# VISION-SJTU/UniDefense

Measured on AMD Instinct MI355X. Metric: images/sec fwd+bwd (256x256, EffNet-b4), higher is better.
Workload: dtype f32

## Files before the change

unidefense_amd/csrc/gemm_p3.hip:

```cpp
#include "gemm_internal.h"
#include "ud_common.h"

#include <algorithm>
#include <type_traits>

namespace {

constexpr int NT = 512;
constexpr int BK = 32;
constexpr int BM = 128, BN = 128;
constexpr int PLANE_IMG = 128 * 64;

template <int PREC> struct Cfg {
    static constexpr int NPL = PREC;
    static constexpr int OP_IMG = NPL * PLANE_IMG;
    static constexpr int STAGE = 2 * OP_IMG;
    static constexpr int NSTAGE = PREC == 3 ? 3 : 4;
    static constexpr int PT = 4 * NPL;
    static constexpr int NTERM = PREC == 3 ? 6 : PREC == 2 ? 3 : 1;
};

typedef __bf16 bf16x8 __attribute__((ext_vector_type(8)));
typedef _Float16 f16x8 __attribute__((ext_vector_type(8)));
typedef short s16x4 __attribute__((ext_vector_type(4)));
typedef short s16x8 __attribute__((ext_vector_type(8)));
typedef __attribute__((address_space(3))) char lds_char;

__device__ __forceinline__ void dma_piece(unsigned voff, unsigned lds_dst, const char* gbase) {
    unsigned keep;
    asm volatile(
        "s_nop 1\n\t"
        "s_mov_b32 %0, m0\n\t"
        "s_mov_b32 m0, %2\n\t"
// ... 10 lines not shown
}
template <int PT>
__device__ __forceinline__ void wait_tiles_and_barrier(int tiles) {
    if (tiles <= 0) wait_dma_and_barrier<0>();
    else if (tiles == 1) wait_dma_and_barrier<PT>();
    else if (tiles == 2) wait_dma_and_barrier<2 * PT>();
    else if (tiles == 3 || PT > 4) wait_dma_and_barrier<3 * PT>();
    else if (tiles == 4) wait_dma_and_barrier<4 * PT>();
    else if (tiles == 5) wait_dma_and_barrier<5 * PT>();
    else wait_dma_and_barrier<6 * PT>();
}
__device__ __forceinline__ void wait_lds_and_barrier() {
    asm volatile("s_waitcnt lgkmcnt(0)\n\ts_barrier" ::: "memory");
}

template <int NPL> struct Frags {
    s16x8 v[2][NPL];
};

template <int MODE>
struct Reader {
    unsigned b0, b1;

    __device__ __forceinline__ void init(int lane, int wrow) {
        if constexpr (MODE == 0) {
            const int r = lane & 31, h = lane >> 5, x = (r >> 2) & 3;
            b0 = (unsigned)((wrow + r) * 64 + ((h ^ x) << 4));
            b1 = (unsigned)((wrow + r) * 64 + (((2 + h) ^ x) << 4));
        } else {
            const int g = lane >> 4, u = lane & 15, q = u >> 2, pp = u & 3;
            b0 = (unsigned)((wrow >> 5) * 2048 + (8 * (g >> 1) + q) * 64 + (g & 1) * 32 + pp * 8);
            b1 = 0;
        }
    }

    template <int S, int I, int PL, int NPL>
    __device__ __forceinline__ void read_one(const lds_char* img, Frags<NPL>& f) const {
        if constexpr (MODE == 0) {
            const lds_char* p = img + (S == 0 ? b0 : b1) + I * 2048 + PL * PLANE_IMG;
            f.v[I][PL] = *reinterpret_cast<const __attribute__((address_space(3))) s16x8*>(p);
        } else {
            const lds_char* p = img + b0 + S * 1024 + I * 2048 + PL * PLANE_IMG;
            const s16x4 lo = __builtin_amdgcn_ds_read_tr16_b64_v4i16((__attribute__((address_space(3))) s16x4*)(p));
            const s16x4 hi = __builtin_amdgcn_ds_read_tr16_b64_v4i16((__attribute__((address_space(3))) s16x4*)(p + 256));
            f.v[I][PL] = __builtin_shufflevector(lo, hi, 0, 1, 2, 3, 4, 5, 6, 7);
        }
    }

    template <int S, int NPL>
    __device__ __forceinline__ void read(const lds_char* img, Frags<NPL>& f) const {
        read_one<S, 0, 0>(img, f); read_one<S, 1, 0>(img, f);
        if constexpr (NPL >= 2) { read_one<S, 0, 1>(img, f); read_one<S, 1, 1>(img, f); }
        if constexpr (NPL == 3) { read_one<S, 0, 2>(img, f); read_one<S, 1, 2>(img, f); }
    }
};

template <int MODE>
__device__ __forceinline__ unsigned dma_lane_offset(int lane) {
    if constexpr (MODE == 0) return (unsigned)((lane >> 2) * 64 + (((lane & 3) ^ ((lane >> 4) & 3)) << 4));
    else return (unsigned)(lane * 16);
}

template <int PREC, int TERM> struct Term {
    static constexpr int pa = PREC == 3 ? (TERM == 0 ? 2 : (TERM == 1 || TERM >= 4) ? 0 : 1) : PREC == 2 ? (TERM == 0 ? 1 : 0) : 0;
    static constexpr int pb = PREC == 3 ? (TERM == 0 ? 0 : TERM == 1 ? 2 : (TERM == 2 || TERM == 4) ? 1 : 0) : PREC == 2 ? (TERM == 1 ? 1 : 0) : 0;
};

template <int PREC, int Mi>
__device__ __forceinline__ void mma_one(f32x16 (&acc)[2][2], f32x16 (&lo)[2][2], const Frags<PREC>& a, const Frags<PREC>& b) {
    constexpr int term = Mi / 4, i = (Mi % 4) / 2, j = Mi % 2;
    using Tm = Term<PREC, term>;
    if constexpr (PREC == 3) {
        acc[i][j] = __builtin_amdgcn_mfma_f32_32x32x16_bf16(__builtin_bit_cast(bf16x8, a.v[i][Tm::pa]),
                                                            __builtin_bit_cast(bf16x8, b.v[j][Tm::pb]), acc[i][j], 0, 0, 0);
    } else if constexpr (PREC == 1) {
        acc[i][j] = __builtin_amdgcn_mfma_f32_32x32x16_f16(__builtin_bit_cast(f16x8, a.v[i][0]),
                                                           __builtin_bit_cast(f16x8, b.v[j][0]), acc[i][j], 0, 0, 0);
    } else if constexpr (term < 2) {
        lo[i][j] = __builtin_amdgcn_mfma_f32_32x32x16_f16(__builtin_bit_cast(f16x8, a.v[i][Tm::pa]),
                                                          __builtin_bit_cast(f16x8, b.v[j][Tm::pb]), lo[i][j], 0, 0, 0);
    } else {
        acc[i][j] = __builtin_amdgcn_mfma_f32_32x32x16_f16(__builtin_bit_cast(f16x8, a.v[i][Tm::pa]),
                                                           __builtin_bit_cast(f16x8, b.v[j][Tm::pb]), acc[i][j], 0, 0, 0);
    }
}

template <int PREC, int AMODE, int BMODE, bool SK>
__device__ __forceinline__ void p3_body(const ud_gemm_p3_desc& d, int tiles_m, int tiles_n, char* L, int bx, int by, int gx) {
    using CF = Cfg<PREC>;
    constexpr int NPL = CF::NPL, OP_IMG = CF::OP_IMG, STAGE = CF::STAGE, NSTAGE = CF::NSTAGE, PT = CF::PT;

    const int tid = threadIdx.x, lane = tid & 63;
    const int wave = __builtin_amdgcn_readfirstlane(tid >> 6);
    const int wm = (wave >> 1) & 1, wn = wave & 1;
    const int l31 = lane & 31, half = lane >> 5;
    const int kt_total = d.K / BK;
    const int dM = d.M, dN = d.N;
    const long ldc = d.ldc;
    const bool c_half = d.c_half != 0;
    double* const stat_sum = d.stat_sum;
    double* const stat_sumsq = d.stat_sumsq;
    const float* const a_inv = d.a_inv_scale;
    const float* const b_inv = d.b_inv_scale;
    const long ast = d.a_scale_stride, bst = d.b_scale_stride;
    const lds_char* Lp = (const lds_char*)L;
    const unsigned lds0 = (unsigned)(uintptr_t)Lp;
    const int lw = wave & 3;
    const unsigned dst_w = lds0 + (unsigned)lw * 2048u;
    const long a_plane = d.a_plane * 2, b_plane = d.b_plane * 2;
    const unsigned a_voff = dma_lane_offset<AMODE>(lane), b_voff = dma_lane_offset<BMODE>(lane);
    Reader<AMODE> ra;
    Reader<BMODE> rb;
    ra.init(lane, wm * 64);
    rb.init(lane, wn * 64);
    using std::integral_constant;
    using H0 = integral_constant<int, 0>;
    using H1 = integral_constant<int, 1>;
    using T = std::true_type;
    using F = std::false_type;

    auto segment = [&](int tile_m, int tile_n, int kt0, int nkt, int ep, float* Cp, bool first) {
        const int m0 = tile_m * BM, n0 = tile_n * BN;
        f32x16 acc[2][2], lo[PREC == 2 ? 2 : 1][2];
#pragma unroll
        for (int i = 0; i < 2; ++i)
#pragma unroll
            for (int j = 0; j < 2; ++j)
#pragma unroll
                for (int r = 0; r < 16; ++r) {
                    acc[i][j][r] = 0.f;
                    if constexpr (PREC == 2) lo[i][j][r] = 0.f;
                }

        if (nkt > 0) {
            if (wave >= 4) {
                const char* a_g0;
                const char* b_g0;
                long a_step, b_step;
                if constexpr (AMODE == 0) {
                    a_g0 = reinterpret_cast<const char*>(d.A) + (long)kt0 * d.a_panel * 2 + (long)(m0 + 32 * lw) * 64;
                    a_step = d.a_panel * 2;
                } else {
                    a_g0 = reinterpret_cast<const char*>(d.A) + (long)min(m0 / 32 + lw, d.a_npanel - 1) * d.a_panel * 2 +
                           (long)kt0 * BK * 64;
                    a_step = BK * 64;
                }
                if constexpr (BMODE == 0) {
                    b_g0 = reinterpret_cast<const char*>(d.B) + (long)kt0 * d.b_panel * 2 + (long)(n0 + 32 * lw) * 64;
                    b_step = d.b_panel * 2;
                } else {
                    b_g0 = reinterpret_cast<const char*>(d.B) + (long)min(n0 / 32 + lw, d.b_npanel - 1) * d.b_panel * 2 +
                           (long)kt0 * BK * 64;
                    b_step = BK * 64;
                }
                auto issue = [&](int t) {
                    const unsigned dst = dst_w + (unsigned)(t % NSTAGE) * STAGE;
                    const char* ga = a_g0 + (long)t * a_step;
                    const char* gb = b_g0 + (long)t * b_step;
#pragma unroll
                    for (int pl = 0; pl < NPL; ++pl)
#pragma unroll
                        for (int jj = 0; jj < 2; ++jj)
                            dma_piece(a_voff, dst + pl * PLANE_IMG + jj * 1024, ga + pl * a_plane + jj * 1024);
#pragma unroll
                    for (int pl = 0; pl < NPL; ++pl)
#pragma unroll
                        for (int jj = 0; jj < 2; ++jj)
                            dma_piece(b_voff, dst + OP_IMG + pl * PLANE_IMG + jj * 1024, gb + pl * b_plane + jj * 1024);
                };
                if (!first) wait_dma_and_barrier<0>();
                const int pro = min(nkt, NSTAGE);
                for (int t = 0; t < pro; ++t) issue(t);
                wait_tiles_and_barrier<PT>(pro - 1);
                for (int t = 0; t + 1 < nkt; ++t) {
                    wait_tiles_and_barrier<PT>(min(nkt, t + NSTAGE) - (t + 2));
                    if (t + NSTAGE < nkt) issue(t + NSTAGE);
                }
                return;
            }
            if (!first) wait_lds_and_barrier();
            wait_lds_and_barrier();

            f32x16 (&lo2)[2][2] = *reinterpret_cast<f32x16 (*)[2][2]>(&lo[0][0]);
            Frags<NPL> fa0, fb0, fa1, fb1;
            ra.template read<0>(Lp, fa0);
            rb.template read<0>(Lp + OP_IMG, fb0);

            auto phase = [&](auto rs_c, auto do_read_c, const Frags<NPL>& ca, const Frags<NPL>& cb, Frags<NPL>& na, Frags<NPL>& nb,
                             const lds_char* img) {
                constexpr int RS = decltype(rs_c)::value;
                constexpr bool RD = decltype(do_read_c)::value;
                constexpr int NSLOT = 2 * NPL, PER = 4 * CF::NTERM / NSLOT;
                auto slot = [&](auto k_c) {
                    constexpr int k = decltype(k_c)::value;
                    constexpr int ai = k & 1, bi = k & 1;
                    constexpr int apl = NPL == 3 ? (k < 2 ? 2 : k < 4 ? 0 : 1) : NPL == 2 ? (k < 2 ? 1 : 0) : 0;
                    constexpr int bpl = NPL == 3 ? (k < 2 ? 0 : k < 4 ? 2 : 1) : NPL == 2 ? (k < 2 ? 0 : 1) : 0;
                    if constexpr (RD) {
                        ra.template read_one<RS, ai, apl>(img, na);
                        rb.template read_one<RS, bi, bpl>(img + OP_IMG, nb);
                    }
                    mma_one<PREC, PER * k>(acc, lo2, ca, cb);
                    mma_one<PREC, PER * k + 1>(acc, lo2, ca, cb);
                    if constexpr (PER >= 3) mma_one<PREC, PER * k + 2>(acc, lo2, ca, cb);
                    if constexpr (PER == 4) mma_one<PREC, PER * k + 3>(acc, lo2, ca, cb);
                    __builtin_amdgcn_sched_barrier(0);
                };
                slot(integral_constant<int, 0>{}); slot(integral_constant<int, 1>{});
                if constexpr (NSLOT >= 4) { slot(integral_constant<int, 2>{}); slot(integral_constant<int, 3>{}); }
                if constexpr (NSLOT == 6) { slot(integral_constant<int, 4>{}); slot(integral_constant<int, 5>{}); }
            };
            for (int t = 0; t + 1 < nkt; ++t) {
                phase(H1{}, T{}, fa0, fb0, fa1, fb1, Lp + (t % NSTAGE) * STAGE);
                wait_lds_and_barrier();
                phase(H0{}, T{}, fa1, fb1, fa0, fb0, Lp + ((t + 1) % NSTAGE) * STAGE);
            }
            phase(H1{}, T{}, fa0, fb0, fa1, fb1, Lp + ((nkt - 1) % NSTAGE) * STAGE);
            phase(H0{}, F{}, fa1, fb1, fa0, fb0, Lp);
        } else if (wave >= 4) {
            return;
        }

        if (nkt <= 0 && ep != 0) return;
        if constexpr (PREC <= 2) {
            const float* __restrict__ as = a_inv;
            const float* __restrict__ bs = b_inv;
            float ib[2], ia[2][16];
#pragma unroll
            for (int j = 0; j < 2; ++j) ib[j] = bs[(long)min(n0 + wn * 64 + j * 32 + l31, dN - 1) * bst];
            if (ast == 0) {
                const float a0 = as[0];
#pragma unroll
                for (int i = 0; i < 2; ++i)
#pragma unroll
                    for (int r = 0; r < 16; ++r) ia[i][r] = a0;
            } else {
#pragma unroll
                for (int i = 0; i < 2; ++i)
#pragma unroll
                    for (int r = 0; r < 16; ++r)
                        ia[i][r] = as[min(m0 + wm * 64 + i * 32 + (r & 3) + 8 * (r >> 2) + 4 * half, dM - 1)];
            }
#pragma unroll
            for (int j = 0; j < 2; ++j) {
                const bool cok = n0 + wn * 64 + j * 32 + l31 < dN;
#pragma unroll
                for (int i = 0; i < 2; ++i)
#pragma unroll
                    for (int r = 0; r < 16; ++r) {
                        const int row = m0 + wm * 64 + i * 32 + (r & 3) + 8 * (r >> 2) + 4 * half;
                        float v = acc[i][j][r];
                        if constexpr (PREC == 2) v += 0x1p-11f * lo[i][j][r];
                        v *= ia[i][r] * ib[j];
                        asm volatile("" : "+v"(v));
                        acc[i][j][r] = (cok && row < dM) ? v : 0.f;
                    }
            }
        }
        if (!SK && stat_sum) {
            if (PREC == 3 && m0 + BM > dM) {
#pragma unroll
                for (int i = 0; i < 2; ++i)
#pragma unroll
                    for (int r = 0; r < 16; ++r) {
                        const int row = m0 + wm * 64 + i * 32 + (r & 3) + 8 * (r >> 2) + 4 * half;
                        if (row >= dM) { acc[i][0][r] = 0.f; acc[i][1][r] = 0.f; }
                    }
            }
            const long slot = (tiles_m > 64) ? (long)(tile_m & 63) * dN : 0;
#pragma unroll
            for (int j = 0; j < 2; ++j) {
                double s1 = 0.0, s2 = 0.0;
#pragma unroll
                for (int i = 0; i < 2; ++i)
#pragma unroll
                    for (int r = 0; r < 16; ++r) {
                        const double v = (double)acc[i][j][r];
                        s1 += v;
                        s2 += v * v;
                    }
                s1 += __shfl_xor(s1, 32, 64);
                s2 += __shfl_xor(s2, 32, 64);
                const int col = n0 + wn * 64 + j * 32 + l31;
                if (half == 0 && col < dN) {
                    unsafeAtomicAdd(stat_sum + slot + col, s1);
                    unsafeAtomicAdd(stat_sumsq + slot + col, s2);
                }
            }
        }
        auto store_all = [&](auto mode_c, auto inside_c) {
            constexpr int MODE = decltype(mode_c)::value;
            constexpr bool INSIDE = decltype(inside_c)::value;
#pragma unroll
            for (int i = 0; i < 2; ++i) {
#pragma unroll
                for (int j = 0; j < 2; ++j) {
                    const int col = n0 + wn * 64 + j * 32 + l31;
                    const long off0 = (long)(m0 + wm * 64 + i * 32 + 4 * half) * ldc + col;
                    float* pc = Cp + off0;
#pragma unroll
                    for (int r = 0; r < 16; ++r) {
                        const int dr = (r & 3) + 8 * (r >> 2);
                        if (INSIDE || (m0 + wm * 64 + i * 32 + 4 * half + dr < dM && col < dN)) {
                            const float v = acc[i][j][r];
                            if constexpr (MODE >= 4) {
                                _Float16* p = reinterpret_cast<_Float16*>(Cp) + off0 + (long)dr * ldc;
                                *p = (_Float16)(MODE == 4 ? v : v + (float)*p);
                            } else {
                                float* p = pc + (long)dr * ldc;
                                if constexpr (MODE == 0) *p = v;
                                else if constexpr (MODE == 1) *p += v;
                                else atomicAdd(p, v);
                            }
                        }
                    }
                }
            }
        };
        const bool inside = m0 + BM <= dM && n0 + BN <= dN;
        if (PREC == 1 && c_half) {
            if (inside) {
                if (ep == 0) store_all(integral_constant<int, 4>{}, T{});
                else store_all(integral_constant<int, 5>{}, T{});
            } else {
                if (ep == 0) store_all(integral_constant<int, 4>{}, F{});
                else store_all(integral_constant<int, 5>{}, F{});
            }
        } else if (inside) {
            if (ep == 0) store_all(integral_constant<int, 0>{}, T{});
            else if (ep == 1) store_all(integral_constant<int, 1>{}, T{});
            else store_all(integral_constant<int, 2>{}, T{});
        } else {
            if (ep == 0) store_all(integral_constant<int, 0>{}, F{});
            else if (ep == 1) store_all(integral_constant<int, 1>{}, F{});
// ... 28 lines not shown
        bool first = true;
        while (u < u1) {
            const int tile = (int)(u / kt_total), kt_b = (int)(u - (long)tile * kt_total);
            const int kt_e = (int)min((long)kt_total, kt_b + (u1 - u));
            const int band = tile / band_tiles, in_band = tile - band * band_tiles;
            const int bw = min(8, tiles_n - band * 8);
            const int tile_m = in_band / bw, tile_n = band * 8 + in_band - tile_m * bw;
            const bool whole = kt_b == 0 && kt_e == kt_total;
            segment(tile_m, tile_n, kt_b, kt_e - kt_b, whole ? d.out_mode : 2, d.C, first);
            first = false;
            u += kt_e - kt_b;
        }
    }
}

template <int PREC, int AMODE, int BMODE, bool SK = false>
__global__ __launch_bounds__(NT, 1) void gemm_p3_kernel(const ud_gemm_p3_desc d, int tiles_m, int tiles_n) {
    using CF = Cfg<PREC>;
    __shared__ __attribute__((aligned(1024))) char L[CF::NSTAGE * CF::STAGE];
    p3_body<PREC, AMODE, BMODE, SK>(d, tiles_m, tiles_n, L, (int)blockIdx.x, (int)blockIdx.y, (int)gridDim.x);
}

template <int PREC, int A0 = 0, int B0 = 1, int A1 = 1, int B1 = 1>
__global__ __launch_bounds__(NT, 1) void gemm_p3_pair_kernel(const ud_gemm_p3_desc d0, int tm0, int tn0, int n0,
                                                              const ud_gemm_p3_desc d1, int tm1, int tn1) {
    using CF = Cfg<PREC>;
    __shared__ __attribute__((aligned(1024))) char L[CF::NSTAGE * CF::STAGE];
    const int b = (int)blockIdx.x;
    const bool first = b < (n0 < 0 ? -n0 : n0);
    const int l = first ? b : b - (n0 < 0 ? -n0 : n0);
    if (first == (n0 > 0)) {
        const int T = tm0 * tn0;
        p3_body<PREC, A0, B0, false>(d0, tm0, tn0, L, l % T, l / T, T);
    } else {
        const int T = tm1 * tn1;
        p3_body<PREC, A1, B1, false>(d1, tm1, tn1, L, l % T, l / T, T);
    }
}

int num_cus() {
    static const int n = [] {
        int dev = 0, cus = 0;
        if (hipGetDevice(&dev) != hipSuccess ||
            hipDeviceGetAttribute(&cus, hipDeviceAttributeMultiprocessorCount, dev) != hipSuccess || cus < 8)
            cus = 256;
        return cus;
    }();
    return n;
}

template <int PREC, int AMODE, int BMODE>
int launch(const ud_gemm_p3_desc& d, hipStream_t s) {
    const int tiles_m = ud_cdiv(d.M, BM), tiles_n = ud_cdiv(d.N, BN);
    if (d.tile_cfg & 0x800) {
        const long U = (long)tiles_m * tiles_n * (d.K / BK);
        long G = std::min<long>(num_cus(), U / 4);
        G = std::max<long>(8, G / 8 * 8);
        hipLaunchKernelGGL((gemm_p3_kernel<PREC, AMODE, BMODE, true>), dim3((unsigned)G), dim3(NT), 0, s, d, tiles_m, tiles_n);
    } else {
        dim3 grid((unsigned)(tiles_m * tiles_n), (unsigned)d.split_k, 1);
        hipLaunchKernelGGL((gemm_p3_kernel<PREC, AMODE, BMODE>), grid, dim3(NT), 0, s, d, tiles_m, tiles_n);
    }
    UD_LAUNCH_CHECK();
    return 0;
}

__device__ __forceinline__ uint32_t pack_bf16(float x, float y) {
// ... 393 lines not shown
    hipLaunchKernelGGL(split_h2_rows_kernel, dim3((unsigned)ud_cdiv(R, 4)), dim3(256), 0, (hipStream_t)stream, x, R, C, ld,
                       planes, panel_stride, plane_stride, inv_scale);
    UD_LAUNCH_CHECK();
    return 0;
}

static bool p3_desc_ok(const ud_gemm_p3_desc& d);

extern "C" int ud_gemm_p3_pair(const ud_gemm_p3_desc* nn, const ud_gemm_p3_desc* tn, ud_stream_t stream) {
    if (!nn || !tn || !p3_desc_ok(*nn) || !p3_desc_ok(*tn)) return UD_EINVAL;
    const ud_gemm_p3_desc &d0 = *nn, &d1 = *tn;
    const bool grads = d0.a_mode == 0 && d0.b_mode == 1 && d1.a_mode == 1 && d1.b_mode == 1;
    const bool tailp = d0.a_mode == 0 && d0.b_mode == 0 && d1.a_mode == 0 && d1.b_mode == 0 && d0.prec == 2;
    if ((d0.prec != 2 && d0.prec != 1) || d1.prec != d0.prec || !(grads || tailp)) return UD_EINVAL;
    if ((d0.tile_cfg | d1.tile_cfg) & 0x800) return UD_EINVAL;
    if (d0.stat_sum || d1.stat_sum || d0.out_mode == 3 || d1.out_mode == 3) return UD_EINVAL;
    const int tm0 = ud_cdiv(d0.M, BM), tn0 = ud_cdiv(d0.N, BN), tm1 = ud_cdiv(d1.M, BM), tn1 = ud_cdiv(d1.N, BN);
    const long n0 = (long)tm0 * tn0 * d0.split_k, n1 = (long)tm1 * tn1 * d1.split_k;
    if (n0 + n1 > 0x7fffffffL) return UD_EINVAL;
    const int nfirst = (d1.tile_cfg & 0x10000) ? -(int)n1 : (int)n0;
    if (tailp)
        hipLaunchKernelGGL((gemm_p3_pair_kernel<2, 0, 0, 0, 0>), dim3((unsigned)(n0 + n1)), dim3(NT), 0, (hipStream_t)stream, d0, tm0,
                           tn0, nfirst, d1, tm1, tn1);
    else if (d0.prec == 1)
        hipLaunchKernelGGL((gemm_p3_pair_kernel<1>), dim3((unsigned)(n0 + n1)), dim3(NT), 0, (hipStream_t)stream, d0, tm0, tn0,
                           nfirst, d1, tm1, tn1);
    else
        hipLaunchKernelGGL((gemm_p3_pair_kernel<2>), dim3((unsigned)(n0 + n1)), dim3(NT), 0, (hipStream_t)stream, d0, tm0, tn0,
                           nfirst, d1, tm1, tn1);
    UD_LAUNCH_CHECK();
    return 0;
}

static bool p3_desc_ok(const ud_gemm_p3_desc& d) {
    if (!d.A || !d.B || !d.C || d.M <= 0 || d.N <= 0 || d.K <= 0 || d.K % BK != 0 || d.split_k < 1 ||
        d.split_k > d.K / BK || d.out_mode < 0 || d.out_mode > 3 || d.a_mode < 0 || d.a_mode > 1 || d.b_mode < 0 ||
        d.b_mode > 1 || d.a_panel % 8 != 0 || d.b_panel % 8 != 0 || d.a_plane % 8 != 0 || d.b_plane % 8 != 0 ||
        d.a_npanel < 1 || d.b_npanel < 1 || d.prec < 1 || d.prec > 3)
        return false;
    if (d.prec <= 2 && (!d.a_inv_scale || !d.b_inv_scale || d.a_scale_stride < 0 || d.a_scale_stride > 1 ||
                        d.b_scale_stride < 0 || d.b_scale_stride > 1))
        return false;
    if (d.stat_sum && (d.out_mode != 0 || d.split_k != 1 || !d.stat_sumsq || (d.tile_cfg & 0x800))) return false;
    if ((d.tile_cfg & 0x800) && (d.out_mode > 1 || d.split_k != 1)) return false;
    if (d.out_mode == 3 && d.slice_stride < (long)d.M * d.ldc) return false;
    if (d.c_half && (d.prec != 1 || d.out_mode > 1 || d.split_k != 1 || (d.tile_cfg & 0x800))) return false;
    return true;
}

extern "C" int ud_gemm_p3(const ud_gemm_p3_desc* dp, ud_stream_t stream) {
    if (!dp) return UD_EINVAL;
    const ud_gemm_p3_desc& d = *dp;
    if (!p3_desc_ok(d)) return UD_EINVAL;
    hipStream_t s = (hipStream_t)stream;
    if (d.prec == 1) {
        if (d.a_mode == 0 && d.b_mode == 0) return launch<1, 0, 0>(d, s);
        if (d.a_mode == 0 && d.b_mode == 1) return launch<1, 0, 1>(d, s);
        if (d.a_mode == 1 && d.b_mode == 1) return launch<1, 1, 1>(d, s);
        return UD_EINVAL;
    }
// ... 13 lines not shown
```

unidefense_amd/kernels.py:

```python
import ctypes as C
import math
import os

import torch

from . import lib as _lib
from .config import cfg as CFG
from .lib import ConvGeom, GemmDesc, GemmP3Desc

_call = _lib.call

GEMM_PROFILE = None


def _stream():
    return C.c_void_p(torch.cuda.current_stream().cuda_stream)


def _key(ref):
    return ref.device.index


def _p(t):
    if t is None:
# ... 423 lines not shown
    assert A.prec == B.prec or max(A.prec, B.prec) <= 2
    d.prec = min(A.prec, B.prec)
    d.c_half = 1 if Cout.dtype == torch.float16 else 0
    if d.prec <= 2:
        assert (a_mode == 0 or not A.scale_stride) and (b_mode == 0 or not B.scale_stride)
        d.a_inv_scale = A.inv.data_ptr() + 4 * a_row0 * A.scale_stride
        d.b_inv_scale = B.inv.data_ptr()
        d.a_scale_stride, d.b_scale_stride = A.scale_stride, B.scale_stride
    return d


_P3_PAIR = True


def _p3_pair_tn_first(M, N, Kd, pn, pt):
    sp = int(pt[1]) if pt[0] == "split" else 1
    t1 = -(-N // 128) * -(-Kd // 128) * sp
    return M / sp > 2.0 * N and t1 <= 256


def _p3_pair_ok(pn, pt):
    return pn[0] in ("plain", "split", "sk") and pt[0] in ("plain", "split")


def spectral_bwd(ctx, dy2, out=None, dy_absmax=None):
    if (ctx.plans is None or not _P3_PAIR or CFG.deterministic or GEMM_PROFILE is not None or
            not _p3_pair_ok(ctx.plans["nn"], ctx.plans["tn"])):
        dw = spectral_wgrad(ctx, dy2, dy_absmax)
        return spectral_dgrad(ctx, dy2, out=out, dy_absmax=dy_absmax), dw
    dy = _spectral_dy(ctx, dy2, dy_absmax)
    pn, pt = ctx.plans["nn"], ctx.plans["tn"]
    if pn[0] == "sk":
        pn = ("plain",)
    M, N, Kd = ctx.M, ctx.N, ctx.K
    acc = out is not None
    if pn[0] == "plain":
        dx = out if acc else empty((M, Kd), dy2, torch.float16 if dy2.dtype == torch.float16 else torch.float32)
        d0 = _p3_desc(dy, ctx.w, dx, M, Kd, -(-N // 32) * 32, 0, 1, 1 if acc else 0, 1)
    else:
        dx = out if acc else split_out((M, Kd), dy2)
        d0 = _p3_desc(dy, ctx.w, dx, M, Kd, -(-N // 32) * 32, 0, 1, 2, int(pn[1]))
    if pt[0] == "plain":
        dw = empty((N, Kd), dy2)
        d1 = _p3_desc(dy, ctx.x, dw, N, Kd, -(-M // 32) * 32, 1, 1, 0, 1)
    else:
        dw = split_out((N, Kd), dy2)
        d1 = _p3_desc(dy, ctx.x, dw, N, Kd, -(-M // 32) * 32, 1, 1, 2, int(pt[1]))
    if _p3_pair_tn_first(M, N, Kd, pn, pt):
        d1.tile_cfg |= 0x10000
    _call("ud_gemm_p3_pair", C.byref(d0), C.byref(d1), _stream())
    return dx, dw


def _gemm_p3(A, B, Cout, M, N, K, a_mode, b_mode, out_mode=0, split_k=1, stats=None, a_row0=0, cfg=0):
    d = _p3_desc(A, B, Cout, M, N, K, a_mode, b_mode, out_mode, split_k, a_row0, cfg)
    slices = None
    if CFG.deterministic and out_mode == 2:
        total = M * N
        fresh = getattr(Cout, "_ud_fresh", False)
        ws = _slice_ws(Cout, split_k * total)
        d.C, d.out_mode, d.slice_stride = ws.data_ptr(), 3, total
        slices = (ws, total, total, 0 if fresh else 1)
# ... 250 lines not shown
        return _gemm(a, w, out, M, N, K, K, N, N, 0, 1, 1 if acc else 0)
    if out is None or accumulate:
        acc = out is not None
        r = _tuned_launch("nn", a, w, out, M, N, K, K, N, 0, 1, acc, None,
                          lambda scr: _model_plan_launch(a, w, scr, M, N, K, K, N, 1, True))
        if r is not None:
            return r
        return _model_plan_launch(a, w, out, M, N, K, K, N, 1, acc)
    return _gemm(a, w, out, M, N, K, K, N, N, 0, 1, 0)


_P2_MIN = (1024, 512)
_P2_SPLITS = (2, 3, 4, 6, 8)
_P2_TN_SPLITS = (1, 2, 3, 4, 6, 8, 12, 16, 24, 32, 48, 64, 96, 128, 192, 256)
_P2_MODES = {"nt": (0, 0), "nn": (0, 1), "tn": (1, 1)}


def _p2_shape_ok(M, N, K):
    return M % 32 == 0 and K % 4 == 0 and N % 4 == 0 and min(N, K) >= 64 and M >= 128


def _p2_plans(kind, M, N, K):
    tiles = -(-M // 128) * -(-N // 128)
    out = []
    if kind == "tn":
        for s_ in _P2_TN_SPLITS:
            if (s_ == 1 or K // 32 // s_ >= 4) and 64 <= tiles * s_ <= 2048:
                out.append(("split", s_) if s_ > 1 else ("plain",))
    else:
        out.append(("plain",))
        for s_ in _P2_SPLITS:
            if K // 32 // s_ >= 4 and tiles * s_ <= 2048:
                out.append(("split", s_))
        tp = _tail_plan(M, N, K)
        if tp is not None:
            out.append(("tail", tp[0], tp[1]))
        if kind == "nt" and not CFG.deterministic:
            out += [("tailp", m1, s_) for m1, s_ in _tailp_plans(M, N, K)]
    if not CFG.deterministic:
        out.append(("sk",))
    return out or [("plain",)]


def _tailp_plans(M, N, K):
    if M < 256 or N < 128 or K < 256:
        return []
    mt, nt = -(-M // 128), -(-N // 128)
    full, tail = divmod(mt * nt, 256)
    if full < 1 or tail == 0:
        return []
    out = []
    for extra in (0, 1):
        rows_tail = -(-tail // nt) + extra
# ... 4 lines not shown
            if K // 32 // s_ >= 4:
                out.append(((mt - rows_tail) * 128, s_))
    return out


def _p2_run(kind, plan, ap, bp, M, N, K, like, stats=None, out=None):
    am, bm = _P2_MODES[kind]
    Kp = -(-K // 32) * 32
    how = plan[0]
    if how == "tailp" and GEMM_PROFILE is not None:
        how = "tail"
    acc = out is not None
    assert not (acc and stats is not None)
    odt = torch.float16 if (like.dtype == torch.float16 and kind != "tn") else torch.float32
    assert odt == torch.float32 or how == "plain"
    if how == "plain":
        return _gemm_p3(ap, bp, out if acc else empty((M, N), like, odt), M, N, Kp, am, bm, 1 if acc else 0, 1, stats=stats)
    res = None
    if how == "split":
        res = _gemm_p3(ap, bp, out if acc else split_out((M, N), like), M, N, Kp, am, bm, 2, int(plan[1]))
    elif how == "sk":
        res = _gemm_p3(ap, bp, out if acc else zeros((M, N), like), M, N, Kp, am, bm, 1 if acc else 0, 1, cfg=0x800)
    elif how == "tailp":
        m1, s_ = int(plan[1]), int(plan[2])
        assert kind == "nt"
        res = out if acc else empty((M, N), like)
        tail = res[m1:]
        if not acc:
            tail.zero_()
        d0 = _p3_desc(ap, bp, res, m1, N, Kp, am, bm, 1 if acc else 0, 1)
        d1 = _p3_desc(ap, bp, tail, M - m1, N, Kp, am, bm, 2, s_, a_row0=m1)
        _call("ud_gemm_p3_pair", C.byref(d0), C.byref(d1), _stream())
    else:
        m1, s_ = int(plan[1]), int(plan[2])
        res = out if acc else empty((M, N), like)
# ... 9 lines not shown


def _p2_default_plan(kind, M, N, K):
    tiles = -(-M // 128) * -(-N // 128)
    if kind == "tn":
        s_ = max(1, min(256 // tiles if tiles <= 256 else 1, K // 32 // 4))
        return ("split", s_) if s_ > 1 else ("plain",)
    full, rem = divmod(tiles, 256)
    if full >= 1 and 0 < rem <= 64:
        tp = _tail_plan(M, N, K)
        if tp is not None:
            return ("tail", tp[0], tp[1])
        if not CFG.deterministic:
            return ("sk",)
    if tiles < 128 and K >= 1024:
        return ("split", min(4, max(2, 256 // tiles)))
    return ("plain",)


_HALF_LIKE = {}


def _half_like(t):
    h = _HALF_LIKE.get(t.device)
    if h is None:
        h = _HALF_LIKE[t.device] = torch.empty(0, dtype=torch.float16, device=t.device)
    return h


def spectral_takes_plane_half(M, N, Kd):
    return _p1_plans_for(M, N, Kd) is not None
# ... 129 lines not shown

    def fwd_x3():
        r = gemm_nt(x2, w2, stats=acc)
        if want_stats and not r[1]:
            colstats(r[0], acc)
    t_x3 = _time_launches(lambda: (fwd_x3(), gemm_nn(dy2, w2), gemm_tn(dy2, x2)))
    xp, wp, dp = split_planes(x2, prec=2), split_planes(w2, prec=2), split_planes(dy2, prec=2)
    t_p2 = _time_launches(lambda: (split_planes(x2, xp), split_planes(dy2, dp), split_planes(w2, wp)))
    t_stats = _time_launches(lambda: colstats(dy2, acc)) if want_stats else 0.0
    plans = []
    for kind, (a, b, m, n, k) in (("nt", (xp, wp, M, N, Kd)), ("nn", (dp, wp, M, Kd, N)), ("tn", (dp, xp, N, Kd, M))):
        best, best_t = None, 1e30
        for plan in _p2_plans(kind, m, n, k):
            st = acc if (kind == "nt" and want_stats) else None
            t = _time_launches(lambda: _p2_run(kind, plan, a, b, m, n, k, x2, stats=st))
            if st is not None and plan[0] != "plain":
                t += t_stats
            if t < best_t:
                best, best_t = plan, t
        plans.append(list(best))
        t_p2 += best_t
    res = plans if (forced or t_p2 < 0.97 * t_x3) else None
    _TUNED[key] = res
    _tune_cache_save()
    return res


_WG_SPLIT_MAXT = 512
_WG_SPLIT_TARGET = 768
_WG_SPLIT_ROWS = 256

# ... 1850 lines not shown
```

Before: 1400.

## Add 64x64 small-tile variant of precision-2 split GEMM kernel for low-tile-count shapes

Adds a templated small-tile (64x64) mode to the split-plane GEMM kernel, selected by a new tile_cfg flag. It covers plain, split-K and paired launches and raises occupancy via launch bounds. The Python planner adds 'small' and 'small_split' candidates to autotuning, and the default plan for small-tile-count, large-K shapes now uses the small tile instead of split-K. The aim is to fill more CUs on small GEMMs without split-K reduction overhead, at the cost of lower data reuse per tile.

```diff
diff --git a/unidefense_amd/csrc/gemm_p3.hip b/unidefense_amd/csrc/gemm_p3.hip
--- a/unidefense_amd/csrc/gemm_p3.hip
+++ b/unidefense_amd/csrc/gemm_p3.hip
@@ -11,12 +11,15 @@
 constexpr int BM = 128, BN = 128;
 constexpr int PLANE_IMG = 128 * 64;
 
-template <int PREC> struct Cfg {
+template <int PREC, bool SM = false> struct Cfg {
     static constexpr int NPL = PREC;
-    static constexpr int OP_IMG = NPL * PLANE_IMG;
+    static constexpr int TBM = SM ? 64 : BM, TBN = SM ? 64 : BN;
+    static constexpr int NRB = SM ? 1 : 2;
+    static constexpr int PIMG = SM ? 64 * 64 : PLANE_IMG;
+    static constexpr int OP_IMG = NPL * PIMG;
     static constexpr int STAGE = 2 * OP_IMG;
     static constexpr int NSTAGE = PREC == 3 ? 3 : 4;
-    static constexpr int PT = 4 * NPL;
+    static constexpr int PT = (SM ? 2 : 4) * NPL;
     static constexpr int NTERM = PREC == 3 ? 6 : PREC == 2 ? 3 : 1;
 };
 
@@ -57,8 +60,9 @@
     asm volatile("s_waitcnt lgkmcnt(0)\n\ts_barrier" ::: "memory");
 }
 
-template <int NPL> struct Frags {
-    s16x8 v[2][NPL];
+template <int NPL, int NRB_ = 2> struct Frags {
+    static constexpr int NRB = NRB_;
+    s16x8 v[NRB_][NPL];
 };
 
 template <int MODE>
@@ -77,24 +81,28 @@
         }
     }
 
-    template <int S, int I, int PL, int NPL>
-    __device__ __forceinline__ void read_one(const lds_char* img, Frags<NPL>& f) const {
+    template <int S, int I, int PL, int PIMG, class FR>
+    __device__ __forceinline__ void read_one(const lds_char* img, FR& f) const {
         if constexpr (MODE == 0) {
-            const lds_char* p = img + (S == 0 ? b0 : b1) + I * 2048 + PL * PLANE_IMG;
+            const lds_char* p = img + (S == 0 ? b0 : b1) + I * 2048 + PL * PIMG;
             f.v[I][PL] = *reinterpret_cast<const __attribute__((address_space(3))) s16x8*>(p);
         } else {
-            const lds_char* p = img + b0 + S * 1024 + I * 2048 + PL * PLANE_IMG;
+            const lds_char* p = img + b0 + S * 1024 + I * 2048 + PL * PIMG;
             const s16x4 lo = __builtin_amdgcn_ds_read_tr16_b64_v4i16((__attribute__((address_space(3))) s16x4*)(p));
             const s16x4 hi = __builtin_amdgcn_ds_read_tr16_b64_v4i16((__attribute__((address_space(3))) s16x4*)(p + 256));
             f.v[I][PL] = __builtin_shufflevector(lo, hi, 0, 1, 2, 3, 4, 5, 6, 7);
         }
     }
 
-    template <int S, int NPL>
-    __device__ __forceinline__ void read(const lds_char* img, Frags<NPL>& f) const {
-        read_one<S, 0, 0>(img, f); read_one<S, 1, 0>(img, f);
-        if constexpr (NPL >= 2) { read_one<S, 0, 1>(img, f); read_one<S, 1, 1>(img, f); }
-        if constexpr (NPL == 3) { read_one<S, 0, 2>(img, f); read_one<S, 1, 2>(img, f); }
+    template <int S, int PIMG, int NPL, int NRB>
+    __device__ __forceinline__ void read(const lds_char* img, Frags<NPL, NRB>& f) const {
+        read_one<S, 0, 0, PIMG>(img, f);
+        if constexpr (NRB == 2) read_one<S, 1, 0, PIMG>(img, f);
+        if constexpr (NPL >= 2) {
+            read_one<S, 0, 1, PIMG>(img, f);
+            if constexpr (NRB == 2) read_one<S, 1, 1, PIMG>(img, f);
+        }
+        if constexpr (NPL == 3) { read_one<S, 0, 2, PIMG>(img, f); read_one<S, 1, 2, PIMG>(img, f); }
     }
 };
 
@@ -109,9 +117,10 @@
     static constexpr int pb = PREC == 3 ? (TERM == 0 ? 0 : TERM == 1 ? 2 : (TERM == 2 || TERM == 4) ? 1 : 0) : PREC == 2 ? (TERM == 1 ? 1 : 0) : 0;
 };
 
-template <int PREC, int Mi>
-__device__ __forceinline__ void mma_one(f32x16 (&acc)[2][2], f32x16 (&lo)[2][2], const Frags<PREC>& a, const Frags<PREC>& b) {
-    constexpr int term = Mi / 4, i = (Mi % 4) / 2, j = Mi % 2;
+template <int PREC, int Mi, int NRB>
+__device__ __forceinline__ void mma_one(f32x16 (&acc)[NRB][NRB], f32x16 (&lo)[NRB][NRB], const Frags<PREC, NRB>& a,
+                                        const Frags<PREC, NRB>& b) {
+    constexpr int NB = NRB * NRB, term = Mi / NB, i = (Mi % NB) / NRB, j = Mi % NRB;
     using Tm = Term<PREC, term>;
     if constexpr (PREC == 3) {
         acc[i][j] = __builtin_amdgcn_mfma_f32_32x32x16_bf16(__builtin_bit_cast(bf16x8, a.v[i][Tm::pa]),
@@ -128,10 +137,12 @@
     }
 }
 
-template <int PREC, int AMODE, int BMODE, bool SK>
+template <int PREC, int AMODE, int BMODE, bool SK, bool SM = false>
 __device__ __forceinline__ void p3_body(const ud_gemm_p3_desc& d, int tiles_m, int tiles_n, char* L, int bx, int by, int gx) {
-    using CF = Cfg<PREC>;
+    static_assert(!SM || (PREC == 2 && !SK), "the small tile: PREC 2, no stream-K");
+    using CF = Cfg<PREC, SM>;
     constexpr int NPL = CF::NPL, OP_IMG = CF::OP_IMG, STAGE = CF::STAGE, NSTAGE = CF::NSTAGE, PT = CF::PT;
+    constexpr int PIMG = CF::PIMG, NRB = CF::NRB, TBM = CF::TBM, TBN = CF::TBN, WR = 32 * NRB;
 
     const int tid = threadIdx.x, lane = tid & 63;
     const int wave = __builtin_amdgcn_readfirstlane(tid >> 6);
@@ -149,13 +160,13 @@
     const lds_char* Lp = (const lds_char*)L;
     const unsigned lds0 = (unsigned)(uintptr_t)Lp;
     const int lw = wave & 3;
-    const unsigned dst_w = lds0 + (unsigned)lw * 2048u;
+    const unsigned dst_w = lds0 + (unsigned)lw * (SM ? 1024u : 2048u);
     const long a_plane = d.a_plane * 2, b_plane = d.b_plane * 2;
     const unsigned a_voff = dma_lane_offset<AMODE>(lane), b_voff = dma_lane_offset<BMODE>(lane);
     Reader<AMODE> ra;
     Reader<BMODE> rb;
-    ra.init(lane, wm * 64);
-    rb.init(lane, wn * 64);
+    ra.init(lane, wm * WR);
+    rb.init(lane, wn * WR);
     using std::integral_constant;
     using H0 = integral_constant<int, 0>;
     using H1 = integral_constant<int, 1>;
@@ -163,12 +174,12 @@
     using F = std::false_type;
 
     auto segment = [&](int tile_m, int tile_n, int kt0, int nkt, int ep, float* Cp, bool first) {
-        const int m0 = tile_m * BM, n0 = tile_n * BN;
-        f32x16 acc[2][2], lo[PREC == 2 ? 2 : 1][2];
-#pragma unroll
-        for (int i = 0; i < 2; ++i)
-#pragma unroll
-            for (int j = 0; j < 2; ++j)
+        const int m0 = tile_m * TBM, n0 = tile_n * TBN;
+        f32x16 acc[NRB][NRB], lo[PREC == 2 ? NRB : 1][NRB];
+#pragma unroll
+        for (int i = 0; i < NRB; ++i)
+#pragma unroll
+            for (int j = 0; j < NRB; ++j)
 #pragma unroll
                 for (int r = 0; r < 16; ++r) {
                     acc[i][j][r] = 0.f;
@@ -180,36 +191,40 @@
                 const char* a_g0;
                 const char* b_g0;
                 long a_step, b_step;
+                constexpr int LR = SM ? 16 : 32;
+                const int lpan = SM ? lw >> 1 : lw;
+                const long lhalf = SM ? (lw & 1) * 1024 : 0;
                 if constexpr (AMODE == 0) {
-                    a_g0 = reinterpret_cast<const char*>(d.A) + (long)kt0 * d.a_panel * 2 + (long)(m0 + 32 * lw) * 64;
+                    a_g0 = reinterpret_cast<const char*>(d.A) + (long)kt0 * d.a_panel * 2 + (long)(m0 + LR * lw) * 64;
                     a_step = d.a_panel * 2;
                 } else {
-                    a_g0 = reinterpret_cast<const char*>(d.A) + (long)min(m0 / 32 + lw, d.a_npanel - 1) * d.a_panel * 2 +
-                           (long)kt0 * BK * 64;
+                    a_g0 = reinterpret_cast<const char*>(d.A) + (long)min(m0 / 32 + lpan, d.a_npanel - 1) * d.a_panel * 2 +
+                           (long)kt0 * BK * 64 + lhalf;
                     a_step = BK * 64;
                 }
                 if constexpr (BMODE == 0) {
-                    b_g0 = reinterpret_cast<const char*>(d.B) + (long)kt0 * d.b_panel * 2 + (long)(n0 + 32 * lw) * 64;
+                    b_g0 = reinterpret_cast<const char*>(d.B) + (long)kt0 * d.b_panel * 2 + (long)(n0 + LR * lw) * 64;
                     b_step = d.b_panel * 2;
                 } else {
-                    b_g0 = reinterpret_cast<const char*>(d.B) + (long)min(n0 / 32 + lw, d.b_npanel - 1) * d.b_panel * 2 +
-                           (long)kt0 * BK * 64;
+                    b_g0 = reinterpret_cast<const char*>(d.B) + (long)min(n0 / 32 + lpan, d.b_npanel - 1) * d.b_panel * 2 +
+                           (long)kt0 * BK * 64 + lhalf;
                     b_step = BK * 64;
                 }
                 auto issue = [&](int t) {
                     const unsigned dst = dst_w + (unsigned)(t % NSTAGE) * STAGE;
                     const char* ga = a_g0 + (long)t * a_step;
                     const char* gb = b_g0 + (long)t * b_step;
+                    constexpr int NJ = SM ? 1 : 2;
 #pragma unroll
                     for (int pl = 0; pl < NPL; ++pl)
 #pragma unroll
-                        for (int jj = 0; jj < 2; ++jj)
-                            dma_piece(a_voff, dst + pl * PLANE_IMG + jj * 1024, ga + pl * a_plane + jj * 1024);
+                        for (int jj = 0; jj < NJ; ++jj)
+                            dma_piece(a_voff, dst + pl * PIMG + jj * 1024, ga + pl * a_plane + jj * 1024);
 #pragma unroll
                     for (int pl = 0; pl < NPL; ++pl)
 #pragma unroll
-                        for (int jj = 0; jj < 2; ++jj)
-                            dma_piece(b_voff, dst + OP_IMG + pl * PLANE_IMG + jj * 1024, gb + pl * b_plane + jj * 1024);
+                        for (int jj = 0; jj < NJ; ++jj)
+                            dma_piece(b_voff, dst + OP_IMG + pl * PIMG + jj * 1024, gb + pl * b_plane + jj * 1024);
                 };
                 if (!first) wait_dma_and_barrier<0>();
                 const int pro = min(nkt, NSTAGE);
@@ -224,29 +239,39 @@
             if (!first) wait_lds_and_barrier();
             wait_lds_and_barrier();
 
-            f32x16 (&lo2)[2][2] = *reinterpret_cast<f32x16 (*)[2][2]>(&lo[0][0]);
-            Frags<NPL> fa0, fb0, fa1, fb1;
-            ra.template read<0>(Lp, fa0);
-            rb.template read<0>(Lp + OP_IMG, fb0);
-
-            auto phase = [&](auto rs_c, auto do_read_c, const Frags<NPL>& ca, const Frags<NPL>& cb, Frags<NPL>& na, Frags<NPL>& nb,
-                             const lds_char* img) {
+            f32x16 (&lo2)[NRB][NRB] = *reinterpret_cast<f32x16 (*)[NRB][NRB]>(&lo[0][0]);
+            using FR = Frags<NPL, NRB>;
+            FR fa0, fb0, fa1, fb1;
+            ra.template read<0, PIMG>(Lp, fa0);
+            rb.template read<0, PIMG>(Lp + OP_IMG, fb0);
+
+            auto phase = [&](auto rs_c, auto do_read_c, const FR& ca, const FR& cb, FR& na, FR& nb, const lds_char* img) {
                 constexpr int RS = decltype(rs_c)::value;
                 constexpr bool RD = decltype(do_read_c)::value;
-                constexpr int NSLOT = 2 * NPL, PER = 4 * CF::NTERM / NSLOT;
+                constexpr int NSLOT = SM ? 2 : 2 * NPL, PER = 4 * CF::NTERM / (2 * NPL);
                 auto slot = [&](auto k_c) {
                     constexpr int k = decltype(k_c)::value;
-                    constexpr int ai = k & 1, bi = k & 1;
-                    constexpr int apl = NPL == 3 ? (k < 2 ? 2 : k < 4 ? 0 : 1) : NPL == 2 ? (k < 2 ? 1 : 0) : 0;
-                    constexpr int bpl = NPL == 3 ? (k < 2 ? 0 : k < 4 ? 2 : 1) : NPL == 2 ? (k < 2 ? 0 : 1) : 0;
+                    constexpr int ai = SM ? 0 : k & 1, bi = ai;
+                    constexpr int kp = SM ? 2 * k : k;
+                    constexpr int apl = NPL == 3 ? (kp < 2 ? 2 : kp < 4 ? 0 : 1) : NPL == 2 ? (kp < 2 ? 1 : 0) : 0;
+                    constexpr int bpl = NPL == 3 ? (kp < 2 ? 0 : kp < 4 ? 2 : 1) : NPL == 2 ? (kp < 2 ? 0 : 1) : 0;
                     if constexpr (RD) {
-                        ra.template read_one<RS, ai, apl>(img, na);
-                        rb.template read_one<RS, bi, bpl>(img + OP_IMG, nb);
+                        ra.template read_one<RS, ai, apl, PIMG>(img, na);
+                        rb.template read_one<RS, bi, bpl, PIMG>(img + OP_IMG, nb);
                     }
-                    mma_one<PREC, PER * k>(acc, lo2, ca, cb);
-                    mma_one<PREC, PER * k + 1>(acc, lo2, ca, cb);
-                    if constexpr (PER >= 3) mma_one<PREC, PER * k + 2>(acc, lo2, ca, cb);
-                    if constexpr (PER == 4) mma_one<PREC, PER * k + 3>(acc, lo2, ca, cb);
+                    if constexpr (SM) {
+                        if constexpr (k == 0) {
+                            mma_one<PREC, 0, NRB>(acc, lo2, ca, cb);
+                        } else {
+                            mma_one<PREC, 1, NRB>(acc, lo2, ca, cb);
+                            mma_one<PREC, 2, NRB>(acc, lo2, ca, cb);
+                        }
+                    } else {
+                        mma_one<PREC, PER * k, NRB>(acc, lo2, ca, cb);
+                        mma_one<PREC, PER * k + 1, NRB>(acc, lo2, ca, cb);
+                        if constexpr (PER >= 3) mma_one<PREC, PER * k + 2, NRB>(acc, lo2, ca, cb);
+                        if constexpr (PER == 4) mma_one<PREC, PER * k + 3, NRB>(acc, lo2, ca, cb);
+                    }
                     __builtin_amdgcn_sched_barrier(0);
                 };
                 slot(integral_constant<int, 0>{}); slot(integral_constant<int, 1>{});
@@ -268,30 +293,30 @@
         if constexpr (PREC <= 2) {
             const float* __restrict__ as = a_inv;
             const float* __restrict__ bs = b_inv;
-            float ib[2], ia[2][16];
-#pragma unroll
-            for (int j = 0; j < 2; ++j) ib[j] = bs[(long)min(n0 + wn * 64 + j * 32 + l31, dN - 1) * bst];
+            float ib[NRB], ia[NRB][16];
+#pragma unroll
+            for (int j = 0; j < NRB; ++j) ib[j] = bs[(long)min(n0 + wn * WR + j * 32 + l31, dN - 1) * bst];
             if (ast == 0) {
                 const float a0 = as[0];
 #pragma unroll
-                for (int i = 0; i < 2; ++i)
+                for (int i = 0; i < NRB; ++i)
 #pragma unroll
                     for (int r = 0; r < 16; ++r) ia[i][r] = a0;
             } else {
 #pragma unroll
-                for (int i = 0; i < 2; ++i)
+                for (int i = 0; i < NRB; ++i)
 #pragma unroll
                     for (int r = 0; r < 16; ++r)
-                        ia[i][r] = as[min(m0 + wm * 64 + i * 32 + (r & 3) + 8 * (r >> 2) + 4 * half, dM - 1)];
+                        ia[i][r] = as[min(m0 + wm * WR + i * 32 + (r & 3) + 8 * (r >> 2) + 4 * half, dM - 1)];
             }
 #pragma unroll
-            for (int j = 0; j < 2; ++j) {
-                const bool cok = n0 + wn * 64 + j * 32 + l31 < dN;
-#pragma unroll
-                for (int i = 0; i < 2; ++i)
+            for (int j = 0; j < NRB; ++j) {
+                const bool cok = n0 + wn * WR + j * 32 + l31 < dN;
+#pragma unroll
+                for (int i = 0; i < NRB; ++i)
 #pragma unroll
                     for (int r = 0; r < 16; ++r) {
-                        const int row = m0 + wm * 64 + i * 32 + (r & 3) + 8 * (r >> 2) + 4 * half;
+                        const int row = m0 + wm * WR + i * 32 + (r & 3) + 8 * (r >> 2) + 4 * half;
                         float v = acc[i][j][r];
                         if constexpr (PREC == 2) v += 0x1p-11f * lo[i][j][r];
                         v *= ia[i][r] * ib[j];
@@ -301,21 +326,22 @@
             }
         }
         if (!SK && stat_sum) {
-            if (PREC == 3 && m0 + BM > dM) {
-#pragma unroll
-                for (int i = 0; i < 2; ++i)
+            if (PREC == 3 && m0 + TBM > dM) {
+#pragma unroll
+                for (int i = 0; i < NRB; ++i)
 #pragma unroll
                     for (int r = 0; r < 16; ++r) {
-                        const int row = m0 + wm * 64 + i * 32 + (r & 3) + 8 * (r >> 2) + 4 * half;
-                        if (row >= dM) { acc[i][0][r] = 0.f; acc[i][1][r] = 0.f; }
+                        const int row = m0 + wm * WR + i * 32 + (r & 3) + 8 * (r >> 2) + 4 * half;
+                        if (row >= dM) { acc[i][0][r] = 0.f; acc[i][NRB - 1][r] = 0.f; }
                     }
             }
-            const long slot = (tiles_m > 64) ? (long)(tile_m & 63) * dN : 0;
-#pragma unroll
-            for (int j = 0; j < 2; ++j) {
+            const long slot = SM ? ((dM + 127) / 128 > 64 ? (long)((tile_m >> 1) & 63) * dN : 0)
+                                 : (tiles_m > 64) ? (long)(tile_m & 63) * dN : 0;
+#pragma unroll
+            for (int j = 0; j < NRB; ++j) {
                 double s1 = 0.0, s2 = 0.0;
 #pragma unroll
-                for (int i = 0; i < 2; ++i)
+                for (int i = 0; i < NRB; ++i)
 #pragma unroll
                     for (int r = 0; r < 16; ++r) {
                         const double v = (double)acc[i][j][r];
@@ -324,7 +350,7 @@
                     }
                 s1 += __shfl_xor(s1, 32, 64);
                 s2 += __shfl_xor(s2, 32, 64);
-                const int col = n0 + wn * 64 + j * 32 + l31;
+                const int col = n0 + wn * WR + j * 32 + l31;
                 if (half == 0 && col < dN) {
                     unsafeAtomicAdd(stat_sum + slot + col, s1);
                     unsafeAtomicAdd(stat_sumsq + slot + col, s2);
@@ -335,16 +361,16 @@
             constexpr int MODE = decltype(mode_c)::value;
             constexpr bool INSIDE = decltype(inside_c)::value;
 #pragma unroll
-            for (int i = 0; i < 2; ++i) {
-#pragma unroll
-                for (int j = 0; j < 2; ++j) {
-                    const int col = n0 + wn * 64 + j * 32 + l31;
-                    const long off0 = (long)(m0 + wm * 64 + i * 32 + 4 * half) * ldc + col;
+            for (int i = 0; i < NRB; ++i) {
+#pragma unroll
+                for (int j = 0; j < NRB; ++j) {
+                    const int col = n0 + wn * WR + j * 32 + l31;
+                    const long off0 = (long)(m0 + wm * WR + i * 32 + 4 * half) * ldc + col;
                     float* pc = Cp + off0;
 #pragma unroll
                     for (int r = 0; r < 16; ++r) {
                         const int dr = (r & 3) + 8 * (r >> 2);
-                        if (INSIDE || (m0 + wm * 64 + i * 32 + 4 * half + dr < dM && col < dN)) {
+                        if (INSIDE || (m0 + wm * WR + i * 32 + 4 * half + dr < dM && col < dN)) {
                             const float v = acc[i][j][r];
                             if constexpr (MODE >= 4) {
                                 _Float16* p = reinterpret_cast<_Float16*>(Cp) + off0 + (long)dr * ldc;
@@ -360,7 +386,7 @@
                 }
             }
         };
-        const bool inside = m0 + BM <= dM && n0 + BN <= dN;
+        const bool inside = m0 + TBM <= dM && n0 + TBN <= dN;
         if (PREC == 1 && c_half) {
             if (inside) {
                 if (ep == 0) store_all(integral_constant<int, 4>{}, T{});
@@ -419,27 +445,27 @@
     }
 }
 
-template <int PREC, int AMODE, int BMODE, bool SK = false>
-__global__ __launch_bounds__(NT, 1) void gemm_p3_kernel(const ud_gemm_p3_desc d, int tiles_m, int tiles_n) {
-    using CF = Cfg<PREC>;
+template <int PREC, int AMODE, int BMODE, bool SK = false, bool SM = false>
+__global__ __launch_bounds__(NT, SM ? 4 : 1) void gemm_p3_kernel(const ud_gemm_p3_desc d, int tiles_m, int tiles_n) {
+    using CF = Cfg<PREC, SM>;
     __shared__ __attribute__((aligned(1024))) char L[CF::NSTAGE * CF::STAGE];
-    p3_body<PREC, AMODE, BMODE, SK>(d, tiles_m, tiles_n, L, (int)blockIdx.x, (int)blockIdx.y, (int)gridDim.x);
-}
-
-template <int PREC, int A0 = 0, int B0 = 1, int A1 = 1, int B1 = 1>
-__global__ __launch_bounds__(NT, 1) void gemm_p3_pair_kernel(const ud_gemm_p3_desc d0, int tm0, int tn0, int n0,
-                                                              const ud_gemm_p3_desc d1, int tm1, int tn1) {
-    using CF = Cfg<PREC>;
+    p3_body<PREC, AMODE, BMODE, SK, SM>(d, tiles_m, tiles_n, L, (int)blockIdx.x, (int)blockIdx.y, (int)gridDim.x);
+}
+
+template <int PREC, int A0 = 0, int B0 = 1, int A1 = 1, int B1 = 1, bool SM = false>
+__global__ __launch_bounds__(NT, SM ? 4 : 1) void gemm_p3_pair_kernel(const ud_gemm_p3_desc d0, int tm0, int tn0, int n0,
+                                                                       const ud_gemm_p3_desc d1, int tm1, int tn1) {
+    using CF = Cfg<PREC, SM>;
     __shared__ __attribute__((aligned(1024))) char L[CF::NSTAGE * CF::STAGE];
     const int b = (int)blockIdx.x;
     const bool first = b < (n0 < 0 ? -n0 : n0);
     const int l = first ? b : b - (n0 < 0 ? -n0 : n0);
     if (first == (n0 > 0)) {
         const int T = tm0 * tn0;
-        p3_body<PREC, A0, B0, false>(d0, tm0, tn0, L, l % T, l / T, T);
+        p3_body<PREC, A0, B0, false, SM>(d0, tm0, tn0, L, l % T, l / T, T);
     } else {
         const int T = tm1 * tn1;
-        p3_body<PREC, A1, B1, false>(d1, tm1, tn1, L, l % T, l / T, T);
+        p3_body<PREC, A1, B1, false, SM>(d1, tm1, tn1, L, l % T, l / T, T);
     }
 }
 
@@ -456,6 +482,15 @@
 
 template <int PREC, int AMODE, int BMODE>
 int launch(const ud_gemm_p3_desc& d, hipStream_t s) {
+    if constexpr (PREC == 2) {
+        if (d.tile_cfg & 0x400) {
+            const int tm = ud_cdiv(d.M, 64), tn = ud_cdiv(d.N, 64);
+            dim3 grid((unsigned)(tm * tn), (unsigned)d.split_k, 1);
+            hipLaunchKernelGGL((gemm_p3_kernel<2, AMODE, BMODE, false, true>), grid, dim3(NT), 0, s, d, tm, tn);
+            UD_LAUNCH_CHECK();
+            return 0;
+        }
+    }
     const int tiles_m = ud_cdiv(d.M, BM), tiles_n = ud_cdiv(d.N, BN);
     if (d.tile_cfg & 0x800) {
         const long U = (long)tiles_m * tiles_n * (d.K / BK);
@@ -879,12 +914,21 @@
     const bool tailp = d0.a_mode == 0 && d0.b_mode == 0 && d1.a_mode == 0 && d1.b_mode == 0 && d0.prec == 2;
     if ((d0.prec != 2 && d0.prec != 1) || d1.prec != d0.prec || !(grads || tailp)) return UD_EINVAL;
     if ((d0.tile_cfg | d1.tile_cfg) & 0x800) return UD_EINVAL;
+    if ((d0.tile_cfg ^ d1.tile_cfg) & 0x400) return UD_EINVAL;
+    const bool small = (d0.tile_cfg & 0x400) != 0;
+    const int tbm = small ? 64 : BM, tbn = small ? 64 : BN;
     if (d0.stat_sum || d1.stat_sum || d0.out_mode == 3 || d1.out_mode == 3) return UD_EINVAL;
-    const int tm0 = ud_cdiv(d0.M, BM), tn0 = ud_cdiv(d0.N, BN), tm1 = ud_cdiv(d1.M, BM), tn1 = ud_cdiv(d1.N, BN);
+    const int tm0 = ud_cdiv(d0.M, tbm), tn0 = ud_cdiv(d0.N, tbn), tm1 = ud_cdiv(d1.M, tbm), tn1 = ud_cdiv(d1.N, tbn);
     const long n0 = (long)tm0 * tn0 * d0.split_k, n1 = (long)tm1 * tn1 * d1.split_k;
     if (n0 + n1 > 0x7fffffffL) return UD_EINVAL;
     const int nfirst = (d1.tile_cfg & 0x10000) ? -(int)n1 : (int)n0;
-    if (tailp)
+    if (small && tailp)
+        hipLaunchKernelGGL((gemm_p3_pair_kernel<2, 0, 0, 0, 0, true>), dim3((unsigned)(n0 + n1)), dim3(NT), 0, (hipStream_t)stream, d0,
+                           tm0, tn0, nfirst, d1, tm1, tn1);
+    else if (small)
+        hipLaunchKernelGGL((gemm_p3_pair_kernel<2, 0, 1, 1, 1, true>), dim3((unsigned)(n0 + n1)), dim3(NT), 0, (hipStream_t)stream, d0,
+                           tm0, tn0, nfirst, d1, tm1, tn1);
+    else if (tailp)
         hipLaunchKernelGGL((gemm_p3_pair_kernel<2, 0, 0, 0, 0>), dim3((unsigned)(n0 + n1)), dim3(NT), 0, (hipStream_t)stream, d0, tm0,
                            tn0, nfirst, d1, tm1, tn1);
     else if (d0.prec == 1)
@@ -909,6 +953,7 @@
     if (d.stat_sum && (d.out_mode != 0 || d.split_k != 1 || !d.stat_sumsq || (d.tile_cfg & 0x800))) return false;
     if ((d.tile_cfg & 0x800) && (d.out_mode > 1 || d.split_k != 1)) return false;
     if (d.out_mode == 3 && d.slice_stride < (long)d.M * d.ldc) return false;
+    if ((d.tile_cfg & 0x400) && (d.prec != 2 || (d.tile_cfg & 0x800))) return false;
     if (d.c_half && (d.prec != 1 || d.out_mode > 1 || d.split_k != 1 || (d.tile_cfg & 0x800))) return false;
     return true;
 }
diff --git a/unidefense_amd/kernels.py b/unidefense_amd/kernels.py
--- a/unidefense_amd/kernels.py
+++ b/unidefense_amd/kernels.py
@@ -461,12 +461,14 @@
 
 
 def _p3_pair_tn_first(M, N, Kd, pn, pt):
-    sp = int(pt[1]) if pt[0] == "split" else 1
+    sp = int(pt[1]) if pt[0] in ("split", "small_split") else 1
     t1 = -(-N // 128) * -(-Kd // 128) * sp
     return M / sp > 2.0 * N and t1 <= 256
 
 
 def _p3_pair_ok(pn, pt):
+    if pn[0] in ("small", "small_split") or pt[0] in ("small", "small_split"):
+        return pn[0] in ("small", "small_split") and pt[0] in ("small", "small_split")
     return pn[0] in ("plain", "split", "sk") and pt[0] in ("plain", "split")
 
 
@@ -481,18 +483,19 @@
         pn = ("plain",)
     M, N, Kd = ctx.M, ctx.N, ctx.K
     acc = out is not None
-    if pn[0] == "plain":
+    cfg = _P3_SMALL if pn[0] in ("small", "small_split") else 0
+    if pn[0] in ("plain", "small"):
         dx = out if acc else empty((M, Kd), dy2, torch.float16 if dy2.dtype == torch.float16 else torch.float32)
-        d0 = _p3_desc(dy, ctx.w, dx, M, Kd, -(-N // 32) * 32, 0, 1, 1 if acc else 0, 1)
+        d0 = _p3_desc(dy, ctx.w, dx, M, Kd, -(-N // 32) * 32, 0, 1, 1 if acc else 0, 1, cfg=cfg)
     else:
         dx = out if acc else split_out((M, Kd), dy2)
-        d0 = _p3_desc(dy, ctx.w, dx, M, Kd, -(-N // 32) * 32, 0, 1, 2, int(pn[1]))
-    if pt[0] == "plain":
+        d0 = _p3_desc(dy, ctx.w, dx, M, Kd, -(-N // 32) * 32, 0, 1, 2, int(pn[1]), cfg=cfg)
+    if pt[0] in ("plain", "small"):
         dw = empty((N, Kd), dy2)
-        d1 = _p3_desc(dy, ctx.x, dw, N, Kd, -(-M // 32) * 32, 1, 1, 0, 1)
+        d1 = _p3_desc(dy, ctx.x, dw, N, Kd, -(-M // 32) * 32, 1, 1, 0, 1, cfg=cfg)
     else:
         dw = split_out((N, Kd), dy2)
-        d1 = _p3_desc(dy, ctx.x, dw, N, Kd, -(-M // 32) * 32, 1, 1, 2, int(pt[1]))
+        d1 = _p3_desc(dy, ctx.x, dw, N, Kd, -(-M // 32) * 32, 1, 1, 2, int(pt[1]), cfg=cfg)
     if _p3_pair_tn_first(M, N, Kd, pn, pt):
         d1.tile_cfg |= 0x10000
     _call("ud_gemm_p3_pair", C.byref(d0), C.byref(d1), _stream())
@@ -773,6 +776,13 @@
 _P2_SPLITS = (2, 3, 4, 6, 8)
 _P2_TN_SPLITS = (1, 2, 3, 4, 6, 8, 12, 16, 24, 32, 48, 64, 96, 128, 192, 256)
 _P2_MODES = {"nt": (0, 0), "nn": (0, 1), "tn": (1, 1)}
+_P3_SMALL = 0x400
+_P2_SMALL_MAXT = 128
+_P2_SMALL_MINK = 512
+
+
+def _p2_small_ok(M, N, K):
+    return -(-M // 128) * -(-N // 128) <= _P2_SMALL_MAXT and K >= _P2_SMALL_MINK
 
 
 def _p2_shape_ok(M, N, K):
@@ -796,6 +806,12 @@
             out.append(("tail", tp[0], tp[1]))
         if kind == "nt" and not CFG.deterministic:
             out += [("tailp", m1, s_) for m1, s_ in _tailp_plans(M, N, K)]
+    if _p2_small_ok(M, N, K):
+        st = -(-M // 64) * -(-N // 64)
+        out.append(("small",))
+        for s_ in (_P2_TN_SPLITS[1:] if kind == "tn" else _P2_SPLITS[:3]):
+            if K // 32 // s_ >= 4 and st * s_ <= 2048:
+                out.append(("small_split", s_))
     if not CFG.deterministic:
         out.append(("sk",))
     return out or [("plain",)]
@@ -830,11 +846,13 @@
     assert not (acc and stats is not None)
     odt = torch.float16 if (like.dtype == torch.float16 and kind != "tn") else torch.float32
     assert odt == torch.float32 or how == "plain"
-    if how == "plain":
-        return _gemm_p3(ap, bp, out if acc else empty((M, N), like, odt), M, N, Kp, am, bm, 1 if acc else 0, 1, stats=stats)
+    if how in ("plain", "small"):
+        return _gemm_p3(ap, bp, out if acc else empty((M, N), like, odt), M, N, Kp, am, bm, 1 if acc else 0, 1, stats=stats,
+                        cfg=_P3_SMALL if how == "small" else 0)
     res = None
-    if how == "split":
-        res = _gemm_p3(ap, bp, out if acc else split_out((M, N), like), M, N, Kp, am, bm, 2, int(plan[1]))
+    if how in ("split", "small_split"):
+        res = _gemm_p3(ap, bp, out if acc else split_out((M, N), like), M, N, Kp, am, bm, 2, int(plan[1]),
+                       cfg=_P3_SMALL if how == "small_split" else 0)
     elif how == "sk":
         res = _gemm_p3(ap, bp, out if acc else zeros((M, N), like), M, N, Kp, am, bm, 1 if acc else 0, 1, cfg=0x800)
     elif how == "tailp":
@@ -874,7 +892,7 @@
         if not CFG.deterministic:
             return ("sk",)
     if tiles < 128 and K >= 1024:
-        return ("split", min(4, max(2, 256 // tiles)))
+        return ("small",)
     return ("plain",)
 
 
@@ -1034,7 +1052,7 @@
         for plan in _p2_plans(kind, m, n, k):
             st = acc if (kind == "nt" and want_stats) else None
             t = _time_launches(lambda: _p2_run(kind, plan, a, b, m, n, k, x2, stats=st))
-            if st is not None and plan[0] != "plain":
+            if st is not None and plan[0] not in ("plain", "small"):
                 t += t_stats
             if t < best_t:
                 best, best_t = plan, t
```

New measurement: 1401 (median of 2 runs). No clear change (+0.1%).
